# LuxGraph/Lux

Measured on AMD Instinct MI355X. Metric: GTEPS, higher is better.
Workload: dtype fp32; 1 GPU; model=pagerank, graph=rmat27, nv=134217728, ne=2147483648, parallelism=graph-partition x1

## Files before the change

lux_amd/_native_gpu.py:

```python
import ctypes
import os

_DIR = os.path.dirname(os.path.abspath(__file__))
_PATH = os.path.join(_DIR, "liblux_gpu.so")

_lib = None


def lib():
    global _lib
    if _lib is None:
        if not os.path.exists(_PATH):
            raise RuntimeError(
                "liblux_gpu.so not built — run `python build.py --gpu` "
                "(the HIP extension is mandatory on GPU boxes; no fallback)")
        _lib = ctypes.CDLL(_PATH)
        _lib.lux_gpu_scan_partials_size.restype = ctypes.c_uint32
    return _lib


def dp(t):
    if t is None:
        return ctypes.c_void_p(0)
    if isinstance(t, int):
# ... 275 lines not shown
    lib().lux_gpu_pull_slots_stream_iter(
        _u64(stream), _u32(n0), dp(cidx0), _u32(nt), dp(tile0), dp(off0),
        dp(scol0), _u32(n1), dp(cidx1), dp(rng1), _u32(n2), dp(cidx2),
        dp(rng2), dp(col), dp(oldv), dp(acc))


def pull_finish_pr_active(stream, na, active, acc, out, deg, row_left,
                          init_rank):
    lib().lux_gpu_pull_finish_pr_active(_u64(stream), _u32(na), dp(active),
                                        dp(acc), dp(out), dp(deg),
                                        _u32(row_left),
                                        ctypes.c_float(init_rank))


def pull_hot_col(stream, n, col, pos, hcol):
    lib().lux_gpu_pull_hot_col(_u64(stream), _u64(n), dp(col), dp(pos),
                               dp(hcol))


def pull_stream_copy_hot(stream, n0, rng0, off0, col, pos, scol0):
    lib().lux_gpu_pull_stream_copy_hot(_u64(stream), _u32(n0), dp(rng0),
                                       dp(off0), dp(col), dp(pos), dp(scol0))


def pull_hot_apos(stream, na, active, pos, deg, row_left, apos):
    lib().lux_gpu_pull_hot_apos(_u64(stream), _u32(na), dp(active), dp(pos),
                                dp(deg), _u32(row_left), dp(apos))


def pull_hot_scatter(stream, nv, pos, old, gold):
    lib().lux_gpu_pull_hot_scatter(_u64(stream), _u32(nv), dp(pos), dp(old),
                                   dp(gold))


def pull_finish_pr_active_hot(stream, na, active, apos, acc, out, gold, deg,
                              row_left, init_rank):
    lib().lux_gpu_pull_finish_pr_active_hot(
        _u64(stream), _u32(na), dp(active), dp(apos), dp(acc), dp(out),
        dp(gold), dp(deg), _u32(row_left), ctypes.c_float(init_rank))


def pull_slots_stream_hot_iter(stream, n0, cidx0, nt, tile0, off0, scol0, n1,
                               cidx1, rng1, n2, cidx2, rng2, col, gold, acc,
                               lo, hi, k):
    rc = lib().lux_gpu_pull_slots_stream_hot_iter(
        _u64(stream), _u32(n0), dp(cidx0), _u32(nt), dp(tile0), dp(off0),
        dp(scol0), _u32(n1), dp(cidx1), dp(rng1), _u32(n2), dp(cidx2),
        dp(rng2), dp(col), dp(gold), dp(acc), _u32(lo), _u32(hi),
        ctypes.c_int(k))
    if rc != 0:
        raise ValueError(f"pull_slots_stream_hot_iter: unsupported k={k}")


def pull_fill_inactive_pr(stream, vp, row_ptr, out, deg, row_left,
                          init_rank):
    lib().lux_gpu_pull_fill_inactive_pr(_u64(stream), _u32(vp), dp(row_ptr),
                                        dp(out), dp(deg), _u32(row_left),
                                        ctypes.c_float(init_rank))


def cf_als_iter(stream, n0, bin0, n1, bin1, n2, bin2, nbig, bin2v, hubidx,
                gram_scratch, rhs_scratch, row_ptr, col, w, oldv, newv,
                row_left, K, oldv_bf=None):
    lib().lux_gpu_cf_als_iter(
        _u64(stream), _u32(n0), dp(bin0), _u32(n1), dp(bin1), _u32(n2),
        dp(bin2), _u32(nbig), dp(bin2v), dp(hubidx), dp(gram_scratch),
        dp(rhs_scratch), dp(row_ptr), dp(col), dp(w), dp(oldv), dp(oldv_bf),
        dp(newv), _u32(row_left), ctypes.c_int(K))


def frontier_expand(stream, old_dense, in_row_left, in_count, old_seg,
                    qlabels, labels_repair, push_row_ptr, items, counter,
                    max_items):
    lib().lux_gpu_frontier_expand(
        _u64(stream), ctypes.c_int(old_dense), _u32(in_row_left),
        _u32(in_count), dp(old_seg), dp(qlabels), dp(labels_repair),
        dp(push_row_ptr), dp(items), dp(counter), _u32(max_items))


def frontier_expand_auto(stream, verts, in_row_left, seg, qlabels,
                         labels_repair, push_row_ptr, items, counter,
                         max_items):
    lib().lux_gpu_frontier_expand_auto(
        _u64(stream), _u32(verts), _u32(in_row_left), dp(seg), dp(qlabels),
        dp(labels_repair), dp(push_row_ptr), dp(items), dp(counter),
        _u32(max_items))


def frontier_fixup(stream, vp, row_left, capacity, built_dense, snapshot,
                   labels_part, deg_part, new_seg, annex, tmp_seg, meta,
                   item_counter, max_items):
    lib().lux_gpu_frontier_fixup(
        _u64(stream), _u32(vp), _u32(row_left), _u32(capacity),
        ctypes.c_int(built_dense), dp(snapshot), dp(labels_part),
        dp(deg_part), dp(new_seg), dp(annex), dp(tmp_seg), dp(meta),
        dp(item_counter), _u32(max_items))


def push_chunk_scatter(stream, is_min, new_dense, items, counter, max_items,
                       push_row_ptr, push_col, old_labels, snapshot,
                       new_labels, my_row_left, new_seg, capacity,
                       visited_bits=None):
    lib().lux_gpu_push_chunk_scatter(
        _u64(stream), ctypes.c_int(is_min), ctypes.c_int(new_dense),
        dp(items), dp(counter), _u32(max_items), dp(push_row_ptr),
        dp(push_col), dp(old_labels), dp(snapshot), dp(new_labels),
# ... 451 lines not shown
```

lux_amd/engine.py:

```python

import torch

from . import _native_gpu as ng
from . import dist as dx

U32 = torch.int32
U64 = torch.int64
F32 = torch.float32


def _stream():
    return torch.cuda.current_stream().cuda_stream


LLC_BLOCK_SHIFT = 23

PULL_STREAM_DEFAULT = "1"
PULL_HOT_DEFAULT = "1"
PULL_HOT_LDS_DEFAULT = "2048"
HOT_BLOCK_SHIFT = 24


def _bins_for(row_ptr, vp, ep, device, compact=False):
    s = _stream()
    bin0 = torch.empty(max(vp, 1), dtype=U32, device=device)
    bin1 = torch.empty(max(vp, 1), dtype=U32, device=device)
    nbig_max = max(min(vp, ep // 2048 + 1), 1)
    n2_max = ep // 8192 + nbig_max + 1
    bin2 = torch.empty(n2_max * 2, dtype=U32, device=device)
    bin2v = torch.empty(nbig_max, dtype=U32, device=device)
    counters = torch.zeros(4, dtype=U32, device=device)
    ng.build_bins(s, vp, row_ptr, bin0, bin1, bin2, bin2v, counters)
    c = counters.cpu()
    n0, n1, n2, nbig = int(c[0]), int(c[1]), int(c[2]), int(c[3])
    if compact:
        bin0 = bin0[:max(n0, 1)].clone()
        bin1 = bin1[:max(n1, 1)].clone()
        bin2 = bin2[:max(n2 * 2, 1)].clone()
        bin2v = bin2v[:max(nbig, 1)].clone()
    return n0, n1, n2, nbig, bin0, bin1, bin2, bin2v


def run_pull_sweeps(part, mode, oldv, newv, deg, init_rank, subset=None):
    s = _stream()
    blocks = getattr(part, "blocks", None)
    weighted = mode == ng.PULL_MIN_W
    if weighted:
        assert part.weight is not None, "PULL_MIN_W needs part.weight"
        assert not blocks or "weight" in blocks[0], \
            "blocked CSC built without weights: prepare_pull(weighted=True)"
    if blocks:
        for blk in blocks:
            if subset == "local" and not blk["local"]:
                continue
            if subset == "remote" and blk["local"]:
                continue
            if isinstance(subset, tuple) and subset[0] == "peer" \
                    and blk.get("owner") != subset[1]:
                continue
            if weighted:
                ng.pull_iter_w(s, blk["n0"], blk["bin0"], blk["n1"],
                               blk["bin1"], blk["n2"], blk["bin2"],
                               blk["nbig"], blk["bin2v"], blk["row_ptr"],
                               blk["col"], blk["weight"], oldv, newv,
                               part.row_left, row_u32=blk.get("row_u32", 0))
                continue
            ng.pull_iter(s, mode, blk["n0"], blk["bin0"], blk["n1"],
                         blk["bin1"], blk["n2"], blk["bin2"], blk["nbig"],
                         blk["bin2v"], blk["row_ptr"], blk["col"], oldv,
                         newv, deg, part.row_left, init_rank,
                         row_u32=blk.get("row_u32", 0))
    else:
        assert subset is None, "subset sweeps need the blocked CSC"
        if weighted:
            ng.pull_iter_w(s, part.n0, part.bin0, part.n1, part.bin1,
                           part.n2, part.bin2, part.nbig, part.bin2v,
                           part.row_ptr, part.col, part.weight, oldv, newv,
                           part.row_left)
            return
        ng.pull_iter(s, mode, part.n0, part.bin0, part.n1, part.bin1,
                     part.n2, part.bin2, part.nbig, part.bin2v, part.row_ptr,
                     part.col, oldv, newv, deg, part.row_left, init_rank)


def pull_stream_enabled():
    import os
    return os.environ.get("LUX_PULL_STREAM", PULL_STREAM_DEFAULT) != "0"


def pull_hot_enabled():
    import os
    return os.environ.get("LUX_PULL_HOT", PULL_HOT_DEFAULT) != "0"


def pull_hot_lds():
    import os
    k = int(os.environ.get("LUX_PULL_HOT_LDS", PULL_HOT_LDS_DEFAULT))
    if k not in (0, 2048, 4096):
        raise ValueError(f"LUX_PULL_HOT_LDS={k}: 0, 2048 or 4096")
    return k


def run_pull_slots_sweeps(part, oldv, acc, stream=None, hot=False,
                          hot_lds=0):
    s = _stream()
    if stream is None:
        stream = pull_stream_enabled()
    col, scol0 = ("hcol", "hscol0") if hot else ("col", "scol0")
    if stream:
        part.prepare_pull_stream(hot=hot)
        if hot and hot_lds:
            for src in part.slot_srcs:
                ng.pull_slots_stream_hot_iter(
                    s, src["n0"], src["cidx0"], src["nt"], src["tile0"],
                    src["off0"], src["hscol0"], src["n1"], src["cidx1"],
                    src["rng1"], src["n2"], src["cidx2"], src["rng2"],
                    src["hcol"], oldv, acc, src["lo"], src["hi"], hot_lds)
            return
        for src in part.slot_srcs:
            ng.pull_slots_stream_iter(
                s, src["n0"], src["cidx0"], src["nt"], src["tile0"],
                src["off0"], src[scol0], src["n1"], src["cidx1"],
                src["rng1"], src["n2"], src["cidx2"], src["rng2"],
                src[col], oldv, acc)
        return
    for src in part.slot_srcs:
        ng.pull_slots_iter(s, src["n0"], src["cidx0"], src["rng0"],
                           src["n1"], src["cidx1"], src["rng1"], src["n2"],
                           src["cidx2"], src["rng2"], src[col], oldv, acc)


def seed_pull(part, mode, oldv, newv):
    if mode == ng.PULL_PR:
        newv.zero_()
    else:
        newv.copy_(oldv.narrow(0, part.row_left, part.vp))


def run_pull(part, mode, oldv, newv, deg, init_rank, seed=True):
    if seed:
        seed_pull(part, mode, oldv, newv)
    run_pull_sweeps(part, mode, oldv, newv, deg, init_rank)
    if mode == ng.PULL_PR:
        ng.pull_finish_pr(_stream(), part.vp, newv, deg, part.row_left,
                          init_rank)


def partition_bounds(col_end, ne, nparts):
    nv = col_end.numel()
    cap = (ne + nparts - 1) // nparts
    targets = torch.tensor(
        [min(cap * (p + 1), ne) for p in range(nparts)], dtype=U64,
        device=col_end.device)
    cuts = torch.searchsorted(col_end, targets, right=True)
    cuts = cuts.cpu().tolist()
    row_left, row_right = [], []
    v = 0
    for p in range(nparts):
        rl = v
        rr = max(cuts[p] - 1, rl) if p < nparts - 1 else nv - 1
        rr = min(rr, nv - 1)
        if rl >= nv:
            row_left.append(1)
# ... 564 lines not shown
    h = engine._handle
    engine._handle = None
    if h is None:
        return
    if isinstance(h, list):
        for _q, w in h:
            w.wait()
    else:
        h.wait()


def _finalize_full(engine):
    _wait_handle(engine)
    if engine.halo is None:
        return
    p = engine.part
    dx.all_gather_slices(engine.old,
                         engine.old.narrow(0, p.row_left, p.vp),
                         p.verts_all, p.row_left_all, my_index=p.p)


class PagerankEngine:

    def __init__(self, part: GraphPart):
        self.part = part
        device = part.device
        s = _stream()
        deg = torch.zeros(part.nv, dtype=U32, device=device)
        ng.hist_u32(s, part.ep, part.col, deg)
        dx.all_reduce_sum_(deg)
        self.deg = deg
        import os
        want_hot = (dx.world_size() == 1 and pull_hot_enabled()
                    and os.environ.get("LUX_PULL_SLOTS", "1") != "0")
        part.prepare_pull(shift=HOT_BLOCK_SHIFT if want_hot else None)
        rank0 = 1.0 / part.nv
        degf = deg.to(F32)
        self.old = torch.where(deg == 0, torch.full_like(degf, rank0),
                               rank0 / degf.clamp(min=1.0))
        self.init_rank = (1.0 - 0.15) / part.nv
        self._slots = (dx.world_size() == 1
                       and os.environ.get("LUX_PULL_SLOTS", "1") != "0"
                       and part.prepare_pull_slots())
        self._stream_role = bool(self._slots) and pull_stream_enabled()
        self._hot = bool(self._slots) and pull_hot_enabled()
        if self._hot:
            part.prepare_pull_hot(deg)
            self.gold = torch.empty(part.nv, dtype=F32, device=device)
            self._gold_stale = True
        if self._stream_role:
            part.prepare_pull_stream(hot=self._hot)
        self._hot_lds = pull_hot_lds() \
            if self._hot and self._stream_role else 0
        if self._slots:
            self.acc = torch.empty(max(part.na, 1), dtype=F32,
                                   device=device)
            self.new_part = None
            self._inactive_done = False
        else:
            self.new_part = torch.empty(part.vp, dtype=F32, device=device)
        self.cur_part = self.old.narrow(0, part.row_left,
                                        part.vp).clone()
        self._handle = None
        self.halo = _maybe_halo(part)
        self._graph = None
        self._steps = 0

    def _pipelined(self):
        p = self.part
        return dx.world_size() > 1 and p.blocks is not None and p.vp > 0

    def _step_body(self):
        p = self.part
        if self._slots:
            self.acc.zero_()
            run_pull_slots_sweeps(p, self.gold if self._hot else self.old,
                                  self.acc, stream=self._stream_role,
                                  hot=self._hot, hot_lds=self._hot_lds)
            if self._hot:
                ng.pull_finish_pr_active_hot(
                    _stream(), p.na, p.active, p.apos, self.acc, self.old,
                    self.gold, self.deg, p.row_left, self.init_rank)
                return
            ng.pull_finish_pr_active(_stream(), p.na, p.active, self.acc,
                                     self.old, self.deg, p.row_left,
                                     self.init_rank)
            return
        run_pull(p, ng.PULL_PR, self.old, self.new_part, self.deg,
                 self.init_rank)
        self.old.narrow(0, p.row_left, p.vp).copy_(self.new_part)

    def _step_single(self):
        import os
        if self._graph is not None:
            self._graph.replay()
            return
        if self._steps >= 2 and os.environ.get("LUX_HIPGRAPH", "1") \
                == "1" and not os.environ.get("LUX_SYNC_CHECK"):
            try:
                g = torch.cuda.CUDAGraph()
                with torch.cuda.graph(g):
                    self._step_body()
                self._graph = g
                self._graph.replay()
                return
            except Exception as e:
                print(f"[lux] hipGraph capture disabled: {e}")
                os.environ["LUX_HIPGRAPH"] = "0"
        self._step_body()

    def step(self):
        p = self.part
        if not self._pipelined():
            if dx.world_size() > 1:
                run_pull(p, ng.PULL_PR, self.old, self.new_part, self.deg,
                         self.init_rank)
                _publish_async(self, self.new_part).wait()
                return
            self._steps += 1
            if self._hot and self._gold_stale:
                ng.pull_hot_scatter(_stream(), p.nv, p.pos, self.old,
                                    self.gold)
                self._gold_stale = False
            self._step_single()
            if self._slots and not self._inactive_done:
                ng.pull_fill_inactive_pr(_stream(), p.vp, p.row_ptr,
                                         self.old, self.deg, p.row_left,
                                         self.init_rank)
                self._inactive_done = True
                self._gold_stale = self._hot
            return
# ... 112 lines not shown
```

src/gpu/pull.hip:

```cpp
#include "gpu_common.h"

namespace lux {

constexpr V_ID T1 = 32;
constexpr V_ID T2 = 2048;
constexpr V_ID CHUNK_EDGES = 8192;

enum PullMode { PR_SUM = 0, LAB_MIN = 1, LAB_MAX = 2, CF_SGD = 3,
                LAB_MIN_W = 4 };


__global__ void build_bins_kernel(V_ID vp, const E_ID* row_ptr,
                                  V_ID* bin0, V_ID* bin1, uint2* bin2,
                                  V_ID* bin2v, uint32_t* counters) {
  __shared__ uint32_t lcnt[4], lbase[4];
  uint64_t stride = (uint64_t)blockDim.x * gridDim.x;
  for (uint64_t tile = (uint64_t)blockIdx.x * blockDim.x; tile < vp;
       tile += stride) {
    uint64_t v = tile + threadIdx.x;
    if (threadIdx.x < 4) lcnt[threadIdx.x] = 0;
    __syncthreads();
    int my_bin = -1;
    uint32_t lpos = 0, nchunks = 0, lpos_c = 0;
    if (v < vp) {
// ... 77 lines not shown
    if (s == INF_LABEL) return INF_LABEL;
    unsigned long long c = (unsigned long long)s + (uint32_t)w;
    return c > 0xFFFFFFFEull ? 0xFFFFFFFEu : (T)c;
  }
  static __device__ __forceinline__ T comb(T a, T b) { return a < b ? a : b; }
  static __device__ __forceinline__ void atom(T* p, T v) { atomicMin(p, v); }
  static __device__ __forceinline__ T reduce_wave(T v) {
    return wave_reduce_min(v);
  }
};

template <PullMode M>
__device__ __forceinline__ typename Val<M>::T finish(
    typename Val<M>::T acc, typename Val<M>::T own, float init_rank,
    V_ID deg) {
  if (M == PR_SUM) {
    float pr = init_rank + PR_ALPHA * (float)acc;
    return deg != 0 ? pr / (float)deg : pr;
  }
  return Val<M>::comb(acc, own);
}

struct PullArgs {
  const void* row_ptr;
  const V_ID* col;
  const void* oldv;
  void* newv;
  const V_ID* deg;
  V_ID row_left;
  float init_rank;
};

struct PullArgsW : PullArgs {
  const WeightType* wgt;
};

template <int K>
struct PullArgsHot : PullArgs {
  V_ID lo;
};
template <int K>
__device__ __forceinline__ float* hot_prefix() {
  __shared__ float hot[K];
  return hot;
}
template <int K>
__device__ __forceinline__ float hot_load(const float* oldv,
                                          const float* hot, V_ID lo,
                                          V_ID c) {
  V_ID r = c - lo;
  const float* p = r < (V_ID)K ? hot + r : oldv + c;
  return *p;
}

template <PullMode M>
__device__ __forceinline__ void store_result(typename Val<M>::T* slot,
                                             typename Val<M>::T acc) {
  *slot = Val<M>::comb(acc, *slot);
}

template <PullMode M>
__device__ __forceinline__ typename Val<M>::T gather_range(
    const typename Val<M>::T* oldv, const V_ID* col, E_ID j, E_ID e,
    E_ID step) {
  using V = Val<M>;
  using T = typename V::T;
  T a0 = V::ident(), a1 = V::ident(), a2 = V::ident(), a3 = V::ident();
  for (; j + 3 * step < e; j += 4 * step) {
    V_ID c0 = col[j], c1 = col[j + step], c2 = col[j + 2 * step],
         c3 = col[j + 3 * step];
    a0 = V::comb(a0, V::map(oldv[c0]));
    a1 = V::comb(a1, V::map(oldv[c1]));
    a2 = V::comb(a2, V::map(oldv[c2]));
    a3 = V::comb(a3, V::map(oldv[c3]));
  }
  for (; j < e; j += step) a0 = V::comb(a0, V::map(oldv[col[j]]));
  return V::comb(V::comb(a0, a1), V::comb(a2, a3));
}

template <PullMode M>
__device__ __forceinline__ typename Val<M>::T gather_range_w(
    const typename Val<M>::T* oldv, const V_ID* col, const WeightType* wgt,
    E_ID j, E_ID e, E_ID step) {
  using V = Val<M>;
  using T = typename V::T;
  T a0 = V::ident(), a1 = V::ident(), a2 = V::ident(), a3 = V::ident();
  for (; j + 3 * step < e; j += 4 * step) {
    V_ID c0 = col[j], c1 = col[j + step], c2 = col[j + 2 * step],
         c3 = col[j + 3 * step];
    WeightType w0 = wgt[j], w1 = wgt[j + step], w2 = wgt[j + 2 * step],
               w3 = wgt[j + 3 * step];
    a0 = V::comb(a0, V::mapw(oldv[c0], w0));
    a1 = V::comb(a1, V::mapw(oldv[c1], w1));
    a2 = V::comb(a2, V::mapw(oldv[c2], w2));
    a3 = V::comb(a3, V::mapw(oldv[c3], w3));
  }
  for (; j < e; j += step) a0 = V::comb(a0, V::mapw(oldv[col[j]], wgt[j]));
  return V::comb(V::comb(a0, a1), V::comb(a2, a3));
}

template <PullMode M>
__device__ __forceinline__ typename Val<M>::T gather_edges(
    const PullArgs& a, const typename Val<M>::T* oldv, E_ID j, E_ID e,
    E_ID step) {
  return gather_range<M>(oldv, a.col, j, e, step);
}
template <PullMode M>
__device__ __forceinline__ typename Val<M>::T gather_edges(
    const PullArgsW& a, const typename Val<M>::T* oldv, E_ID j, E_ID e,
    E_ID step) {
  return gather_range_w<M>(oldv, a.col, a.wgt, j, e, step);
}
template <PullMode M, int K>
__device__ __forceinline__ float gather_edges(const PullArgsHot<K>& a,
                                              const float* oldv, E_ID j,
                                              E_ID e, E_ID step) {
  static_assert(M == PR_SUM, "hot prefix: float sums only");
  const float* hot = hot_prefix<K>();
  const V_ID* col = a.col;
  V_ID lo = a.lo;
  float a0 = 0.0f, a1 = 0.0f, a2 = 0.0f, a3 = 0.0f;
  for (; j + 3 * step < e; j += 4 * step) {
    V_ID c0 = col[j], c1 = col[j + step], c2 = col[j + 2 * step],
         c3 = col[j + 3 * step];
    a0 = a0 + hot_load<K>(oldv, hot, lo, c0);
    a1 = a1 + hot_load<K>(oldv, hot, lo, c1);
    a2 = a2 + hot_load<K>(oldv, hot, lo, c2);
    a3 = a3 + hot_load<K>(oldv, hot, lo, c3);
  }
  for (; j < e; j += step) a0 = a0 + hot_load<K>(oldv, hot, lo, col[j]);
  return (a0 + a1) + (a2 + a3);
}

__device__ __forceinline__ float old_load(const PullArgs&, const float* oldv,
                                          V_ID c) {
  return oldv[c];
}
template <int K>
__device__ __forceinline__ float old_load(const PullArgsHot<K>& a,
                                          const float* oldv, V_ID c) {
  return hot_load<K>(oldv, hot_prefix<K>(), a.lo, c);
}

template <typename RowT>
struct TableRows {
  const V_ID* bin;
  const RowT* row_ptr;
  __device__ __forceinline__ V_ID row(uint64_t i) const { return bin[i]; }
  __device__ __forceinline__ void range(uint64_t, V_ID v, E_ID& b,
                                        E_ID& e) const {
    b = row_ptr[v];
    e = row_ptr[v + 1];
  }
};
template <typename RowT>
struct TableChunks {
  const uint2* bin2;
  const RowT* row_ptr;
  __device__ __forceinline__ V_ID row(uint64_t i, uint32_t& chunk) const {
    uint2 ent = bin2[i];
    chunk = ent.y;
    return ent.x;
  }
  __device__ __forceinline__ void range(uint64_t, V_ID v, uint32_t chunk,
                                        E_ID& b, E_ID& e) const {
    b = (E_ID)row_ptr[v] + (E_ID)chunk * CHUNK_EDGES;
    e = row_ptr[v + 1];
    if (e > b + CHUNK_EDGES) e = b + CHUNK_EDGES;
  }
};
struct SlotRows {
  const V_ID* cidx;
  const uint2* rng;
  __device__ __forceinline__ V_ID row(uint64_t i) const { return cidx[i]; }
  __device__ __forceinline__ V_ID row(uint64_t i, uint32_t&) const {
    return cidx[i];
  }
  __device__ __forceinline__ void range(uint64_t i, V_ID, E_ID& b,
                                        E_ID& e) const {
    uint2 r = rng[i];
    b = r.x;
    e = r.y;
  }
  __device__ __forceinline__ void range(uint64_t i, V_ID, uint32_t, E_ID& b,
                                        E_ID& e) const {
    range(i, 0, b, e);
  }
};

template <PullMode M, typename Src, typename Args>
__device__ __forceinline__ void pull_thread_role(uint32_t blk, uint32_t nblk,
                                                 uint32_t n0, const Src& src,
                                                 const Args& a) {
  using V = Val<M>;
// ... 106 lines not shown

template <typename RowT>
__global__ void pull_chunk_w_kernel(uint32_t n2, const uint2* bin2,
                                    PullArgsW a) {
  pull_chunk_role<LAB_MIN_W>(blockIdx.x, gridDim.x, n2,
                             TableChunks<RowT>{bin2, (const RowT*)a.row_ptr},
                             a);
}

struct SlotBins {
  uint32_t n0, n1, n2;
  uint32_t g1, g2;
  const V_ID *cidx0, *cidx1, *cidx2;
  const uint2 *rng0, *rng1, *rng2;
};

template <PullMode M>
__global__ void __launch_bounds__(BLOCK)
    pull_slots_kernel(SlotBins s, PullArgs a) {
  uint32_t blk = blockIdx.x;
  if (blk < s.g2) {
    pull_chunk_role<M>(blk, s.g2, s.n2, SlotRows{s.cidx2, s.rng2}, a);
  } else if (blk < s.g2 + s.g1) {
    pull_wave_role<M>(blk - s.g2, s.g1, s.n1, SlotRows{s.cidx1, s.rng1}, a);
  } else {
    pull_thread_role<M>(blk - s.g2 - s.g1, gridDim.x - s.g2 - s.g1, s.n0,
                        SlotRows{s.cidx0, s.rng0}, a);
  }
}

constexpr uint32_t TILE_EDGES = 512;
constexpr uint32_t TILE_GROUP = WAVE;

struct SlotStream {
  uint32_t nt;
  const uint32_t* tile0;
  const uint32_t* off0;
  const V_ID* scol0;
};

__device__ __forceinline__ float lds_range_sum(const float* v, uint32_t j,
                                               uint32_t e) {
  float a0 = 0.0f, a1 = 0.0f, a2 = 0.0f, a3 = 0.0f;
  for (; j + 3 < e; j += 4) {
    a0 = a0 + v[j];
    a1 = a1 + v[j + 1];
    a2 = a2 + v[j + 2];
    a3 = a3 + v[j + 3];
  }
  for (; j < e; j++) a0 = a0 + v[j];
  return (a0 + a1) + (a2 + a3);
}

template <PullMode M, typename Args>
__device__ __forceinline__ void pull_stream_role(uint32_t blk, uint32_t nblk,
                                                 const SlotStream& st,
                                                 const V_ID* cidx0,
                                                 const Args& a) {
  static_assert(M == PR_SUM, "stream role: float sums only");
  constexpr uint32_t NW = BLOCK / WAVE;
  __shared__ float vals[NW][TILE_EDGES];
  const float* oldv = (const float*)a.oldv;
  float* acc = (float*)a.newv;
  uint32_t lane = threadIdx.x & (WAVE - 1);
  uint32_t wid = __builtin_amdgcn_readfirstlane(threadIdx.x >> 6);
  float* v = vals[wid];
  uint64_t nwaves = (uint64_t)nblk * NW;
  uint64_t t = (uint64_t)blk * NW + wid;
  if (t >= st.nt) return;
  uint32_t s0 = st.tile0[t], s1 = st.tile0[t + 1];
  uint32_t e0 = st.off0[s0], e1 = st.off0[s1];
  for (;;) {
    uint64_t tn = t + nwaves;
    bool more = tn < st.nt;
    uint32_t s0n = 0, s1n = 0, e0n = 0, e1n = 0;
    if (more) {
      s0n = st.tile0[tn];
      s1n = st.tile0[tn + 1];
    }
    uint32_t rb = 0, re = 0;
    V_ID ci = 0;
    float prev = 0.0f;
    bool row = lane < s1 - s0;
    if (row) {
      rb = st.off0[s0 + lane] - e0;
      re = st.off0[s0 + lane + 1] - e0;
      ci = cidx0[s0 + lane];
      prev = acc[ci];
    }
    for (uint32_t base = e0 + lane; base < e1; base += 4 * WAVE) {
      uint32_t i0 = base, i1 = base + WAVE, i2 = base + 2 * WAVE,
               i3 = base + 3 * WAVE;
      bool p1 = i1 < e1, p2 = i2 < e1, p3 = i3 < e1;
      V_ID c0 = st.scol0[i0];
      V_ID c1 = p1 ? st.scol0[i1] : 0;
      V_ID c2 = p2 ? st.scol0[i2] : 0;
      V_ID c3 = p3 ? st.scol0[i3] : 0;
      float x0 = old_load(a, oldv, c0);
      float x1 = p1 ? old_load(a, oldv, c1) : 0.0f;
      float x2 = p2 ? old_load(a, oldv, c2) : 0.0f;
      float x3 = p3 ? old_load(a, oldv, c3) : 0.0f;
      v[i0 - e0] = x0;
      if (p1) v[i1 - e0] = x1;
      if (p2) v[i2 - e0] = x2;
      if (p3) v[i3 - e0] = x3;
    }
    if (more) {
      e0n = st.off0[s0n];
      e1n = st.off0[s1n];
    }
    __builtin_amdgcn_fence(__ATOMIC_RELEASE, "wavefront");
    __builtin_amdgcn_wave_barrier();
    __builtin_amdgcn_fence(__ATOMIC_ACQUIRE, "wavefront");
    if (row) acc[ci] = Val<M>::comb(lds_range_sum(v, rb, re), prev);
    __builtin_amdgcn_fence(__ATOMIC_RELEASE, "wavefront");
    __builtin_amdgcn_wave_barrier();
    if (!more) break;
    t = tn;
    s0 = s0n, s1 = s1n, e0 = e0n, e1 = e1n;
  }
}

template <PullMode M>
__global__ void __launch_bounds__(BLOCK)
    pull_slots_stream_kernel(SlotBins s, SlotStream st, PullArgs a) {
  uint32_t blk = blockIdx.x;
  if (blk < s.g2) {
    pull_chunk_role<M>(blk, s.g2, s.n2, SlotRows{s.cidx2, s.rng2}, a);
  } else if (blk < s.g2 + s.g1) {
    pull_wave_role<M>(blk - s.g2, s.g1, s.n1, SlotRows{s.cidx1, s.rng1}, a);
  } else {
    pull_stream_role<M>(blk - s.g2 - s.g1, gridDim.x - s.g2 - s.g1, st,
                        s.cidx0, a);
  }
}

template <PullMode M, int K>
__global__ void __launch_bounds__(BLOCK)
    pull_slots_stream_hot_kernel(SlotBins s, SlotStream st, PullArgsHot<K> a,
                                 V_ID hi) {
  float* hot = hot_prefix<K>();
  const float* oldv = (const float*)a.oldv;
  for (uint32_t i = threadIdx.x; i < (uint32_t)K; i += BLOCK) {
    uint64_t p = (uint64_t)a.lo + i;
    hot[i] = p < hi ? oldv[p] : 0.0f;
  }
  __syncthreads();
  uint32_t blk = blockIdx.x;
  if (blk < s.g2) {
    pull_chunk_role<M>(blk, s.g2, s.n2, SlotRows{s.cidx2, s.rng2}, a);
  } else if (blk < s.g2 + s.g1) {
    pull_wave_role<M>(blk - s.g2, s.g1, s.n1, SlotRows{s.cidx1, s.rng1}, a);
  } else {
    pull_stream_role<M>(blk - s.g2 - s.g1, gridDim.x - s.g2 - s.g1, st,
                        s.cidx0, a);
  }
}


__global__ void pull_active_flags_kernel(V_ID vp, const E_ID* row_ptr,
                                         uint32_t* flags) {
  uint64_t stride = (uint64_t)blockDim.x * gridDim.x;
  for (uint64_t v = blockIdx.x * (uint64_t)blockDim.x + threadIdx.x; v < vp;
       v += stride)
    flags[v] = row_ptr[v + 1] != row_ptr[v];
}

__global__ void pull_active_list_kernel(V_ID vp, const uint32_t* flags,
                                        const E_ID* ends, V_ID* active) {
  uint64_t stride = (uint64_t)blockDim.x * gridDim.x;
  for (uint64_t v = blockIdx.x * (uint64_t)blockDim.x + threadIdx.x; v < vp;
       v += stride)
    if (flags[v]) active[ends[v] - 1] = (V_ID)v;
}

template <typename RowT>
__global__ void pull_build_slots_kernel(uint32_t n, const V_ID* bin,
                                        const RowT* row_ptr, const E_ID* ends,
                                        V_ID* cidx, uint2* rng) {
  uint64_t stride = (uint64_t)blockDim.x * gridDim.x;
  for (uint64_t i = blockIdx.x * (uint64_t)blockDim.x + threadIdx.x; i < n;
       i += stride) {
    V_ID v = bin[i];
    cidx[i] = (V_ID)(ends[v] - 1);
    rng[i] = make_uint2((uint32_t)row_ptr[v], (uint32_t)row_ptr[v + 1]);
  }
}

template <typename RowT>
__global__ void pull_build_hub_slots_kernel(uint32_t n2, const uint2* bin2,
                                            const RowT* row_ptr,
                                            const E_ID* ends, V_ID* cidx,
                                            uint2* rng) {
  TableChunks<RowT> t{bin2, row_ptr};
  uint64_t stride = (uint64_t)blockDim.x * gridDim.x;
  for (uint64_t i = blockIdx.x * (uint64_t)blockDim.x + threadIdx.x; i < n2;
       i += stride) {
    uint32_t chunk;
    V_ID v = t.row(i, chunk);
    E_ID b, e;
    t.range(i, v, chunk, b, e);
    cidx[i] = (V_ID)(ends[v] - 1);
    rng[i] = make_uint2((uint32_t)b, (uint32_t)e);
  }
}


__global__ void pull_slot_counts_kernel(uint32_t n, const uint2* rng,
// ... 352 lines not shown
  hipLaunchKernelGGL(pull_stream_tile_fill_kernel, dim3(grid_for(ngroups)),
                     dim3(BLOCK), 0, (hipStream_t)stream, n0, off0, ends,
                     tile0);
  LUX_POST_LAUNCH(stream);
}

void lux_gpu_pull_slots_stream_iter(
    uint64_t stream, uint32_t n0, const V_ID* cidx0, uint32_t nt,
    const uint32_t* tile0, const uint32_t* off0, const V_ID* scol0,
    uint32_t n1, const V_ID* cidx1, const uint2* rng1, uint32_t n2,
    const V_ID* cidx2, const uint2* rng2, const V_ID* col, const float* oldv,
    float* acc) {
  uint32_t g2 = n2 ? (n2 > (uint32_t)MAX_GRID ? MAX_GRID : n2) : 0;
  uint32_t g1 = n1 ? grid_for((uint64_t)n1 * WAVE) : 0;
  uint32_t g0 = n0 && nt ? grid_for((uint64_t)nt * WAVE) : 0;
  if (g0 + g1 + g2 == 0) return;
  SlotBins sb{n0, n1, n2, g1, g2, cidx0, cidx1, cidx2, nullptr, rng1, rng2};
  SlotStream st{g0 ? nt : 0, tile0, off0, scol0};
  PullArgs a{nullptr, col, oldv, acc, nullptr, 0, 0.0f};
  hipLaunchKernelGGL(pull_slots_stream_kernel<PR_SUM>, dim3(g0 + g1 + g2),
                     dim3(BLOCK), 0, (hipStream_t)stream, sb, st, a);
  LUX_POST_LAUNCH(stream);
}

int lux_gpu_pull_slots_stream_hot_iter(
    uint64_t stream, uint32_t n0, const V_ID* cidx0, uint32_t nt,
    const uint32_t* tile0, const uint32_t* off0, const V_ID* scol0,
    uint32_t n1, const V_ID* cidx1, const uint2* rng1, uint32_t n2,
    const V_ID* cidx2, const uint2* rng2, const V_ID* col, const float* gold,
    float* acc, V_ID lo, V_ID hi, int k) {
  if (k != 2048 && k != 4096) return -1;
  uint32_t g2 = n2 ? (n2 > (uint32_t)MAX_GRID ? MAX_GRID : n2) : 0;
  uint32_t g1 = n1 ? grid_for((uint64_t)n1 * WAVE) : 0;
  uint32_t g0 = n0 && nt ? grid_for((uint64_t)nt * WAVE) : 0;
  if (g0 + g1 + g2 == 0) return 0;
  SlotBins sb{n0, n1, n2, g1, g2, cidx0, cidx1, cidx2, nullptr, rng1, rng2};
  SlotStream st{g0 ? nt : 0, tile0, off0, scol0};
#define LUX_HOT(K_)                                                           \
  do {                                                                        \
    PullArgsHot<K_> a{{nullptr, col, gold, acc, nullptr, 0, 0.0f}, lo};       \
    hipLaunchKernelGGL((pull_slots_stream_hot_kernel<PR_SUM, K_>),            \
                       dim3(g0 + g1 + g2), dim3(BLOCK), 0,                    \
                       (hipStream_t)stream, sb, st, a, hi);                   \
  } while (0)
  switch (k) {
    case 2048: LUX_HOT(2048); break;
    default: LUX_HOT(4096); break;
  }
#undef LUX_HOT
  LUX_POST_LAUNCH(stream);
  return 0;
}

void lux_gpu_pull_finish_pr_active(uint64_t stream, V_ID na,
                                   const V_ID* active, const float* acc,
                                   float* out, const V_ID* deg, V_ID row_left,
                                   float init_rank) {
  if (!na) return;
  hipLaunchKernelGGL(pull_finish_pr_active_kernel, dim3(grid_for(na)),
                     dim3(BLOCK), 0, (hipStream_t)stream, na, active, acc,
                     out, deg, row_left, init_rank);
  LUX_POST_LAUNCH(stream);
}


void lux_gpu_pull_hot_col(uint64_t stream, uint64_t n, const V_ID* col,
                          const V_ID* pos, V_ID* hcol) {
  if (!n) return;
  hipLaunchKernelGGL(pull_hot_col_kernel, dim3(grid_for(n)), dim3(BLOCK), 0,
                     (hipStream_t)stream, n, col, pos, hcol);
  LUX_POST_LAUNCH(stream);
}

void lux_gpu_pull_stream_copy_hot(uint64_t stream, uint32_t n0,
                                  const uint2* rng0, const uint32_t* off0,
                                  const V_ID* col, const V_ID* pos,
                                  V_ID* scol0) {
  if (!n0) return;
  hipLaunchKernelGGL(pull_stream_copy_hot_kernel, dim3(grid_for(n0)),
                     dim3(BLOCK), 0, (hipStream_t)stream, n0, rng0, off0, col,
                     pos, scol0);
  LUX_POST_LAUNCH(stream);
}

void lux_gpu_pull_hot_apos(uint64_t stream, V_ID na, const V_ID* active,
                           const V_ID* pos, const V_ID* deg, V_ID row_left,
                           V_ID* apos) {
  if (!na) return;
  hipLaunchKernelGGL(pull_hot_apos_kernel, dim3(grid_for(na)), dim3(BLOCK), 0,
                     (hipStream_t)stream, na, active, pos, deg, row_left,
                     apos);
  LUX_POST_LAUNCH(stream);
}

void lux_gpu_pull_hot_scatter(uint64_t stream, V_ID nv, const V_ID* pos,
                              const float* old, float* gold) {
  if (!nv) return;
  hipLaunchKernelGGL(pull_hot_scatter_kernel, dim3(grid_for(nv)), dim3(BLOCK),
                     0, (hipStream_t)stream, nv, pos, old, gold);
  LUX_POST_LAUNCH(stream);
}

void lux_gpu_pull_finish_pr_active_hot(uint64_t stream, V_ID na,
                                       const V_ID* active, const V_ID* apos,
                                       const float* acc, float* out,
                                       float* gold, const V_ID* deg,
// ... 21 lines not shown
```

src/include/lux/gpu_api.h:

```cpp
#pragma once
#include <cstdint>

#include "types.h"

#ifndef __HIP_PLATFORM_AMD__
struct lux_uint2 { uint32_t x, y; };
#else
using lux_uint2 = uint2;
#endif

extern "C" {

void lux_gpu_rmat_edges(uint64_t stream, uint64_t seed, int scale,
                        uint64_t ne, lux::V_ID* src, lux::V_ID* dst);
void lux_gpu_rmat_edges_folded(uint64_t stream, uint64_t seed, int scale,
                               lux::V_ID nv, uint64_t ne, lux::V_ID* src,
                               lux::V_ID* dst);
void lux_gpu_bipartite_edges(uint64_t stream, uint64_t seed,
                             lux::V_ID n_users, lux::V_ID n_items,
                             uint64_t ne, lux::V_ID* src, lux::V_ID* dst,
                             lux::WeightType* w);
void lux_gpu_hist_u32(uint64_t stream, uint64_t n, const lux::V_ID* ids,
                      uint32_t* hist);
void lux_gpu_rmat_edges_chunk(uint64_t stream, uint64_t seed, int scale,
// ... 86 lines not shown
                                  lux::V_ID* cidx, lux_uint2* rng);
void lux_gpu_pull_slots_iter(uint64_t stream, uint32_t n0,
                             const lux::V_ID* cidx0, const lux_uint2* rng0,
                             uint32_t n1, const lux::V_ID* cidx1,
                             const lux_uint2* rng1, uint32_t n2,
                             const lux::V_ID* cidx2, const lux_uint2* rng2,
                             const lux::V_ID* col, const float* oldv,
                             float* acc);
void lux_gpu_pull_slot_counts(uint64_t stream, uint32_t n,
                              const lux_uint2* rng, uint32_t* cnt);
void lux_gpu_pull_stream_copy(uint64_t stream, uint32_t n0,
                              const lux_uint2* rng0, const uint32_t* off0,
                              const lux::V_ID* col, lux::V_ID* scol0);
void lux_gpu_pull_stream_tile_counts(uint64_t stream, uint32_t n0,
                                     const uint32_t* off0, uint32_t* cnt);
void lux_gpu_pull_stream_tile_fill(uint64_t stream, uint32_t n0,
                                   const uint32_t* off0,
                                   const lux::E_ID* ends, uint32_t* tile0);
void lux_gpu_pull_slots_stream_iter(
    uint64_t stream, uint32_t n0, const lux::V_ID* cidx0, uint32_t nt,
    const uint32_t* tile0, const uint32_t* off0, const lux::V_ID* scol0,
    uint32_t n1, const lux::V_ID* cidx1, const lux_uint2* rng1, uint32_t n2,
    const lux::V_ID* cidx2, const lux_uint2* rng2, const lux::V_ID* col,
    const float* oldv, float* acc);
void lux_gpu_pull_finish_pr_active(uint64_t stream, lux::V_ID na,
                                   const lux::V_ID* active, const float* acc,
                                   float* out, const lux::V_ID* deg,
                                   lux::V_ID row_left, float init_rank);
void lux_gpu_pull_hot_col(uint64_t stream, uint64_t n, const lux::V_ID* col,
                          const lux::V_ID* pos, lux::V_ID* hcol);
void lux_gpu_pull_stream_copy_hot(uint64_t stream, uint32_t n0,
                                  const lux_uint2* rng0,
                                  const uint32_t* off0, const lux::V_ID* col,
                                  const lux::V_ID* pos, lux::V_ID* scol0);
void lux_gpu_pull_hot_apos(uint64_t stream, lux::V_ID na,
                           const lux::V_ID* active, const lux::V_ID* pos,
                           const lux::V_ID* deg, lux::V_ID row_left,
                           lux::V_ID* apos);
void lux_gpu_pull_hot_scatter(uint64_t stream, lux::V_ID nv,
                              const lux::V_ID* pos, const float* old,
                              float* gold);
void lux_gpu_pull_finish_pr_active_hot(uint64_t stream, lux::V_ID na,
                                       const lux::V_ID* active,
                                       const lux::V_ID* apos,
                                       const float* acc, float* out,
                                       float* gold, const lux::V_ID* deg,
                                       lux::V_ID row_left, float init_rank);
int lux_gpu_pull_slots_stream_hot_iter(
    uint64_t stream, uint32_t n0, const lux::V_ID* cidx0, uint32_t nt,
    const uint32_t* tile0, const uint32_t* off0, const lux::V_ID* scol0,
    uint32_t n1, const lux::V_ID* cidx1, const lux_uint2* rng1, uint32_t n2,
    const lux::V_ID* cidx2, const lux_uint2* rng2, const lux::V_ID* col,
    const float* gold, float* acc, lux::V_ID lo, lux::V_ID hi, int k);
void lux_gpu_pull_fill_inactive_pr(uint64_t stream, lux::V_ID vp,
                                   const lux::E_ID* row_ptr, float* out,
                                   const lux::V_ID* deg, lux::V_ID row_left,
                                   float init_rank);

void lux_gpu_csr_scatter(uint64_t stream, uint64_t ep, const lux::V_ID* col,
                         const lux::E_ID* row_ptr_loc, lux::V_ID vp,
                         lux::V_ID row_left, unsigned long long* cursor,
                         lux::V_ID* push_col);
void lux_gpu_frontier_expand(uint64_t stream, int old_dense,
                             lux::V_ID in_row_left, lux::V_ID in_count,
                             const uint8_t* old_seg,
                             const uint32_t* qlabels ,
                             uint32_t* labels_repair ,
                             const lux::E_ID* push_row_ptr,
                             lux_uint2* items, uint32_t* counter,
                             uint32_t max_items);
void lux_gpu_frontier_expand_auto(uint64_t stream, lux::V_ID verts,
                                  lux::V_ID in_row_left, const uint8_t* seg,
                                  const uint32_t* qlabels,
                                  uint32_t* labels_repair,
                                  const lux::E_ID* push_row_ptr,
                                  lux_uint2* items, uint32_t* counter,
                                  uint32_t max_items);
void lux_gpu_frontier_fixup(uint64_t stream, lux::V_ID vp,
                            lux::V_ID row_left, lux::V_ID capacity,
                            int built_dense, const uint32_t* snapshot,
                            const uint32_t* labels_part,
                            const uint32_t* deg_part, uint8_t* new_seg,
                            uint32_t* annex, uint8_t* tmp_seg,
                            uint32_t* meta,
                            const uint32_t* item_counter ,
                            uint32_t max_items);
void lux_gpu_push_chunk_scatter(uint64_t stream, int is_min, int new_dense,
                                const lux_uint2* items,
                                const uint32_t* counter, uint32_t max_items,
                                const lux::E_ID* push_row_ptr,
                                const lux::V_ID* push_col,
                                const uint32_t* old_labels,
                                const uint32_t* snapshot,
                                uint32_t* new_labels, lux::V_ID my_row_left,
                                uint8_t* new_seg, lux::V_ID capacity,
                                uint32_t* visited_bits );
void lux_gpu_bits_from_labels(uint64_t stream, lux::V_ID vp,
                              const uint32_t* labels, uint32_t* bits);

void lux_gpu_build_bitmap(uint64_t stream, lux::V_ID vp,
                          const uint32_t* snapshot,
                          const uint32_t* new_labels, uint8_t* seg);
void lux_gpu_d2s(uint64_t stream, lux::V_ID vp, lux::V_ID row_left,
                 const uint8_t* dense_seg, uint8_t* sparse_seg);
void lux_gpu_publish_labels_guarded(uint64_t stream, lux::V_ID vp,
                                    const uint32_t* meta,
// ... 277 lines not shown
```

Measured before the change: 152.1 GTEPS.

## Add wide 1024-thread hot pull kernel with larger LDS hot prefix per role

```diff
diff --git a/lux_amd/_native_gpu.py b/lux_amd/_native_gpu.py
--- a/lux_amd/_native_gpu.py
+++ b/lux_amd/_native_gpu.py
@@ -351,6 +351,24 @@
         raise ValueError(f"pull_slots_stream_hot_iter: unsupported k={k}")
 
 
+def pull_slots_stream_hot_wide_iter(stream, n0, cidx0, nt, tile0, off0,
+                                    scol0, n1, cidx1, rng1, n2, cidx2, rng2,
+                                    col, gold, acc, lo, hi, ks, kw,
+                                    max_groups=0):
+    rc = lib().lux_gpu_pull_slots_stream_hot_wide_iter(
+        _u64(stream), _u32(n0), dp(cidx0), _u32(nt), dp(tile0), dp(off0),
+        dp(scol0), _u64(0 if scol0 is None else scol0.numel()), _u32(n1),
+        dp(cidx1), dp(rng1), _u32(n2), dp(cidx2), dp(rng2), dp(col),
+        _u64(col.numel()), dp(gold), dp(acc), _u32(lo), _u32(hi),
+        ctypes.c_int(ks), ctypes.c_int(kw), _u32(max_groups))
+    if rc == -1:
+        raise ValueError("pull_slots_stream_hot_wide_iter: unsupported "
+                         f"(ks, kw)=({ks}, {kw})")
+    if rc != 0:
+        raise RuntimeError("pull_slots_stream_hot_wide_iter: the runtime "
+                           "refused the CU count or the LDS size")
+
+
 def pull_fill_inactive_pr(stream, vp, row_ptr, out, deg, row_left,
                           init_rank):
     lib().lux_gpu_pull_fill_inactive_pr(_u64(stream), _u32(vp), dp(row_ptr),
diff --git a/lux_amd/engine.py b/lux_amd/engine.py
--- a/lux_amd/engine.py
+++ b/lux_amd/engine.py
@@ -18,6 +18,8 @@
 PULL_STREAM_DEFAULT = "1"
 PULL_HOT_DEFAULT = "1"
 PULL_HOT_LDS_DEFAULT = "2048"
+PULL_HOT_WIDE_DEFAULT = "1"
+PULL_HOT_WIDE_PREFIX = (8192, 16384)
 HOT_BLOCK_SHIFT = 24
 
 
@@ -101,14 +103,29 @@
     return k
 
 
+def pull_hot_wide_enabled():
+    import os
+    return os.environ.get("LUX_PULL_HOT_WIDE", PULL_HOT_WIDE_DEFAULT) != "0"
+
+
 def run_pull_slots_sweeps(part, oldv, acc, stream=None, hot=False,
-                          hot_lds=0):
+                          hot_lds=0, hot_wide=None, max_groups=0):
     s = _stream()
     if stream is None:
         stream = pull_stream_enabled()
     col, scol0 = ("hcol", "hscol0") if hot else ("col", "scol0")
     if stream:
         part.prepare_pull_stream(hot=hot)
+        if hot and hot_lds and hot_wide:
+            ks, kw = hot_wide
+            for src in part.slot_srcs:
+                ng.pull_slots_stream_hot_wide_iter(
+                    s, src["n0"], src["cidx0"], src["nt"], src["tile0"],
+                    src["off0"], src["hscol0"], src["n1"], src["cidx1"],
+                    src["rng1"], src["n2"], src["cidx2"], src["rng2"],
+                    src["hcol"], oldv, acc, src["lo"], src["hi"], ks, kw,
+                    max_groups)
+            return
         if hot and hot_lds:
             for src in part.slot_srcs:
                 ng.pull_slots_stream_hot_iter(
@@ -779,6 +796,8 @@
             part.prepare_pull_stream(hot=self._hot)
         self._hot_lds = pull_hot_lds() \
             if self._hot and self._stream_role else 0
+        self._hot_wide = PULL_HOT_WIDE_PREFIX \
+            if self._hot_lds and pull_hot_wide_enabled() else None
         if self._slots:
             self.acc = torch.empty(max(part.na, 1), dtype=F32,
                                    device=device)
@@ -803,7 +822,8 @@
             self.acc.zero_()
             run_pull_slots_sweeps(p, self.gold if self._hot else self.old,
                                   self.acc, stream=self._stream_role,
-                                  hot=self._hot, hot_lds=self._hot_lds)
+                                  hot=self._hot, hot_lds=self._hot_lds,
+                                  hot_wide=self._hot_wide)
             if self._hot:
                 ng.pull_finish_pr_active_hot(
                     _stream(), p.na, p.active, p.apos, self.acc, self.old,
diff --git a/src/gpu/pull.hip b/src/gpu/pull.hip
--- a/src/gpu/pull.hip
+++ b/src/gpu/pull.hip
@@ -153,6 +153,14 @@
   const float* p = r < (V_ID)K ? hot + r : oldv + c;
   return *p;
 }
+template <int K, int OFF>
+struct PullArgsWide : PullArgs {
+  V_ID lo;
+};
+__device__ __forceinline__ float* wide_lds() {
+  extern __shared__ float wide_lds_[];
+  return wide_lds_;
+}
 
 template <PullMode M>
 __device__ __forceinline__ void store_result(typename Val<M>::T* slot,
@@ -212,14 +220,11 @@
     E_ID step) {
   return gather_range_w<M>(oldv, a.col, a.wgt, j, e, step);
 }
-template <PullMode M, int K>
-__device__ __forceinline__ float gather_edges(const PullArgsHot<K>& a,
-                                              const float* oldv, E_ID j,
-                                              E_ID e, E_ID step) {
-  static_assert(M == PR_SUM, "hot prefix: float sums only");
-  const float* hot = hot_prefix<K>();
-  const V_ID* col = a.col;
-  V_ID lo = a.lo;
+template <int K>
+__device__ __forceinline__ float gather_range_hot(const float* oldv,
+                                                  const float* hot, V_ID lo,
+                                                  const V_ID* col, E_ID j,
+                                                  E_ID e, E_ID step) {
   float a0 = 0.0f, a1 = 0.0f, a2 = 0.0f, a3 = 0.0f;
   for (; j + 3 * step < e; j += 4 * step) {
     V_ID c0 = col[j], c1 = col[j + step], c2 = col[j + 2 * step],
@@ -232,6 +237,20 @@
   for (; j < e; j += step) a0 = a0 + hot_load<K>(oldv, hot, lo, col[j]);
   return (a0 + a1) + (a2 + a3);
 }
+template <PullMode M, int K>
+__device__ __forceinline__ float gather_edges(const PullArgsHot<K>& a,
+                                              const float* oldv, E_ID j,
+                                              E_ID e, E_ID step) {
+  static_assert(M == PR_SUM, "hot prefix: float sums only");
+  return gather_range_hot<K>(oldv, hot_prefix<K>(), a.lo, a.col, j, e, step);
+}
+template <PullMode M, int K, int OFF>
+__device__ __forceinline__ float gather_edges(const PullArgsWide<K, OFF>& a,
+                                              const float* oldv, E_ID j,
+                                              E_ID e, E_ID step) {
+  static_assert(M == PR_SUM, "hot prefix: float sums only");
+  return gather_range_hot<K>(oldv, wide_lds() + OFF, a.lo, a.col, j, e, step);
+}
 
 __device__ __forceinline__ float old_load(const PullArgs&, const float* oldv,
                                           V_ID c) {
@@ -241,6 +260,11 @@
 __device__ __forceinline__ float old_load(const PullArgsHot<K>& a,
                                           const float* oldv, V_ID c) {
   return hot_load<K>(oldv, hot_prefix<K>(), a.lo, c);
+}
+template <int K, int OFF>
+__device__ __forceinline__ float old_load(const PullArgsWide<K, OFF>& a,
+                                          const float* oldv, V_ID c) {
+  return hot_load<K>(oldv, wide_lds() + OFF, a.lo, c);
 }
 
 template <typename RowT>
@@ -453,14 +477,13 @@
   return (a0 + a1) + (a2 + a3);
 }
 
-template <PullMode M, typename Args>
-__device__ __forceinline__ void pull_stream_role(uint32_t blk, uint32_t nblk,
-                                                 const SlotStream& st,
-                                                 const V_ID* cidx0,
-                                                 const Args& a) {
+template <PullMode M, uint32_t NW, typename Args>
+__device__ __forceinline__ void pull_stream_tiles(uint32_t blk, uint32_t nblk,
+                                                  const SlotStream& st,
+                                                  const V_ID* cidx0,
+                                                  const Args& a,
+                                                  float (*vals)[TILE_EDGES]) {
   static_assert(M == PR_SUM, "stream role: float sums only");
-  constexpr uint32_t NW = BLOCK / WAVE;
-  __shared__ float vals[NW][TILE_EDGES];
   const float* oldv = (const float*)a.oldv;
   float* acc = (float*)a.newv;
   uint32_t lane = threadIdx.x & (WAVE - 1);
@@ -522,6 +545,16 @@
   }
 }
 
+template <PullMode M, typename Args>
+__device__ __forceinline__ void pull_stream_role(uint32_t blk, uint32_t nblk,
+                                                 const SlotStream& st,
+                                                 const V_ID* cidx0,
+                                                 const Args& a) {
+  constexpr uint32_t NW = BLOCK / WAVE;
+  __shared__ float vals[NW][TILE_EDGES];
+  pull_stream_tiles<M, NW>(blk, nblk, st, cidx0, a, vals);
+}
+
 template <PullMode M>
 __global__ void __launch_bounds__(BLOCK)
     pull_slots_stream_kernel(SlotBins s, SlotStream st, PullArgs a) {
@@ -555,6 +588,83 @@
   } else {
     pull_stream_role<M>(blk - s.g2 - s.g1, gridDim.x - s.g2 - s.g1, st,
                         s.cidx0, a);
+  }
+}
+
+constexpr int WIDE_BLOCK = 1024;
+constexpr uint32_t WIDE_NW = WIDE_BLOCK / WAVE;
+constexpr uint32_t WIDE_Q = WIDE_BLOCK / BLOCK;
+constexpr uint32_t WIDE_TILE_FLOATS = WIDE_NW * TILE_EDGES;
+constexpr uint32_t WIDE_SCRATCH = WIDE_Q * (BLOCK / WAVE);
+constexpr uint32_t WIDE_GROUPS_PER_CU = 8;
+
+template <int KS, int KW>
+constexpr uint32_t wide_lds_bytes() {
+  uint32_t s = WIDE_TILE_FLOATS + KS, w = KW + WIDE_SCRATCH;
+  return 4 * (s > w ? s : w);
+}
+
+template <int K, int OFF>
+__device__ __forceinline__ void pull_chunk_role_wide(
+    uint32_t blk, uint32_t nblk, uint32_t n2, const SlotRows& src,
+    const PullArgsWide<K, OFF>& a, float* scratch) {
+  using V = Val<PR_SUM>;
+  const float* oldv = (const float*)a.oldv;
+  float* newv = (float*)a.newv;
+  uint32_t q = threadIdx.x / BLOCK, tq = threadIdx.x % BLOCK;
+  uint32_t lane = tq & (WAVE - 1), wid = tq >> 6;
+  float* lds = scratch + q * (BLOCK / WAVE);
+  for (uint64_t base = (uint64_t)blk * WIDE_Q; base < n2;
+       base += (uint64_t)nblk * WIDE_Q) {
+    uint64_t i = base + q;
+    bool work = i < n2;
+    V_ID v = 0;
+    if (work) {
+      uint32_t chunk = 0;
+      v = src.row(i, chunk);
+      E_ID b, e;
+      src.range(i, v, chunk, b, e);
+      float acc = gather_edges<PR_SUM>(a, oldv, b + tq, e, BLOCK);
+      acc = V::reduce_wave(acc);
+      if (lane == 0) lds[wid] = acc;
+    }
+    __syncthreads();
+    if (work && tq == 0) {
+      float acc = lds[0];
+      for (int w = 1; w < BLOCK / WAVE; w++) acc = V::comb(acc, lds[w]);
+      V::atom(&newv[v], acc);
+    }
+    __syncthreads();
+  }
+}
+
+template <int KS, int KW>
+__global__ void __launch_bounds__(WIDE_BLOCK, 8)
+    pull_slots_stream_hot_wide_kernel(SlotBins s, SlotStream st, PullArgs p,
+                                      V_ID lo, V_ID hi) {
+  uint32_t blk = blockIdx.x;
+  bool stream = blk >= s.g2 + s.g1;
+  float* hot = wide_lds() + (stream ? WIDE_TILE_FLOATS : 0);
+  uint32_t k = stream ? KS : KW;
+  const float* oldv = (const float*)p.oldv;
+  for (uint32_t i = threadIdx.x; i < k; i += WIDE_BLOCK) {
+    uint64_t pos = (uint64_t)lo + i;
+    hot[i] = pos < hi ? oldv[pos] : 0.0f;
+  }
+  __syncthreads();
+  if (blk < s.g2) {
+    PullArgsWide<KW, 0> a{p, lo};
+    pull_chunk_role_wide(blk, s.g2, s.n2, SlotRows{s.cidx2, s.rng2}, a,
+                         wide_lds() + KW);
+  } else if (!stream) {
+    PullArgsWide<KW, 0> a{p, lo};
+    pull_wave_role<PR_SUM>(blk - s.g2, s.g1, s.n1, SlotRows{s.cidx1, s.rng1},
+                           a);
+  } else {
+    PullArgsWide<KS, WIDE_TILE_FLOATS> a{p, lo};
+    pull_stream_tiles<PR_SUM, WIDE_NW>(
+        blk - s.g2 - s.g1, gridDim.x - s.g2 - s.g1, st, s.cidx0, a,
+        (float(*)[TILE_EDGES])wide_lds());
   }
 }
 
@@ -1013,6 +1123,83 @@
   return 0;
 }
 
+static void wide_split(uint32_t g, const uint64_t edges[3],
+                       const uint64_t work[3], const uint32_t per[3],
+                       uint32_t out[3]) {
+  uint64_t tot = 0;
+  uint32_t roles = 0, sum = 0;
+  for (int r = 0; r < 3; r++)
+    if (work[r]) tot += edges[r] ? edges[r] : 1, roles++;
+  if (g < roles) g = roles;
+  for (int r = 0; r < 3; r++) {
+    uint64_t e = edges[r] ? edges[r] : 1;
+    out[r] = work[r] ? (uint32_t)((double)g * (double)e / (double)tot) : 0;
+    if (work[r] && !out[r]) out[r] = 1;
+    sum += out[r];
+  }
+  while (sum != g) {
+    int big = 0;
+    for (int r = 1; r < 3; r++)
+      if (out[r] > out[big]) big = r;
+    if (sum < g) out[big]++, sum++;
+    else out[big]--, sum--;
+  }
+  for (int r = 0; r < 3; r++) {
+    uint64_t cap = (work[r] + per[r] - 1) / per[r];
+    if (out[r] > cap) out[r] = (uint32_t)cap;
+  }
+}
+
+int lux_gpu_pull_slots_stream_hot_wide_iter(
+    uint64_t stream, uint32_t n0, const V_ID* cidx0, uint32_t nt,
+    const uint32_t* tile0, const uint32_t* off0, const V_ID* scol0,
+    uint64_t ne0, uint32_t n1, const V_ID* cidx1, const uint2* rng1,
+    uint32_t n2, const V_ID* cidx2, const uint2* rng2, const V_ID* col,
+    uint64_t ne, const float* gold, float* acc, V_ID lo, V_ID hi, int ks,
+    int kw, uint32_t max_groups) {
+  if (ks != 8192 || kw != 16384) return -1;
+  uint32_t g = max_groups;
+  if (!g) {
+    static const uint32_t dflt = [] {
+      int dev = 0, cus = 0;
+      if (hipGetDevice(&dev) != hipSuccess ||
+          hipDeviceGetAttribute(&cus, hipDeviceAttributeMultiprocessorCount,
+                                dev) != hipSuccess)
+        return 0u;
+      return (uint32_t)(WIDE_GROUPS_PER_CU * cus);
+    }();
+    if (!dflt) return -2;
+    g = dflt;
+  }
+  uint64_t work[3] = {n2, n1, n0 && nt ? nt : 0};
+  uint64_t e2 = (uint64_t)n2 * CHUNK_EDGES, rest = ne > ne0 ? ne - ne0 : 0;
+  if (e2 > rest) e2 = rest;
+  uint64_t edges[3] = {e2, rest - e2, ne0};
+  uint32_t per[3] = {WIDE_Q, WIDE_NW, WIDE_NW}, gr[3];
+  if (!(work[0] | work[1] | work[2])) return 0;
+  wide_split(g, edges, work, per, gr);
+  uint32_t g2 = gr[0], g1 = gr[1], g0 = gr[2];
+  SlotBins sb{n0, n1, n2, g1, g2, cidx0, cidx1, cidx2, nullptr, rng1, rng2};
+  SlotStream st{g0 ? nt : 0, tile0, off0, scol0};
+  PullArgs a{nullptr, col, gold, acc, nullptr, 0, 0.0f};
+#define LUX_WIDE(KS_, KW_)                                                    \
+  do {                                                                        \
+    auto kern = pull_slots_stream_hot_wide_kernel<KS_, KW_>;                  \
+    constexpr uint32_t bytes = wide_lds_bytes<KS_, KW_>();                    \
+    static_assert(2 * bytes <= 160 * 1024, "two workgroups per CU");          \
+    static const hipError_t raised = hipFuncSetAttribute(                     \
+        (const void*)kern, hipFuncAttributeMaxDynamicSharedMemorySize,        \
+        (int)bytes);                                                          \
+    if (raised != hipSuccess) return -2;                                      \
+    hipLaunchKernelGGL(kern, dim3(g0 + g1 + g2), dim3(WIDE_BLOCK), bytes,     \
+                       (hipStream_t)stream, sb, st, a, lo, hi);               \
+  } while (0)
+  LUX_WIDE(8192, 16384);
+#undef LUX_WIDE
+  LUX_POST_LAUNCH(stream);
+  return 0;
+}
+
 void lux_gpu_pull_finish_pr_active(uint64_t stream, V_ID na,
                                    const V_ID* active, const float* acc,
                                    float* out, const V_ID* deg, V_ID row_left,
diff --git a/src/include/lux/gpu_api.h b/src/include/lux/gpu_api.h
--- a/src/include/lux/gpu_api.h
+++ b/src/include/lux/gpu_api.h
@@ -162,6 +162,13 @@
     uint32_t n1, const lux::V_ID* cidx1, const lux_uint2* rng1, uint32_t n2,
     const lux::V_ID* cidx2, const lux_uint2* rng2, const lux::V_ID* col,
     const float* gold, float* acc, lux::V_ID lo, lux::V_ID hi, int k);
+int lux_gpu_pull_slots_stream_hot_wide_iter(
+    uint64_t stream, uint32_t n0, const lux::V_ID* cidx0, uint32_t nt,
+    const uint32_t* tile0, const uint32_t* off0, const lux::V_ID* scol0,
+    uint64_t ne0, uint32_t n1, const lux::V_ID* cidx1, const lux_uint2* rng1,
+    uint32_t n2, const lux::V_ID* cidx2, const lux_uint2* rng2,
+    const lux::V_ID* col, uint64_t ne, const float* gold, float* acc,
+    lux::V_ID lo, lux::V_ID hi, int ks, int kw, uint32_t max_groups);
 void lux_gpu_pull_fill_inactive_pr(uint64_t stream, lux::V_ID vp,
                                    const lux::E_ID* row_ptr, float* out,
                                    const lux::V_ID* deg, lux::V_ID row_left,
```

New measurement: 156.4 GTEPS (median of 6 runs). 1.03x the previous value.
